# facebookresearch/spdl

Hardware: AMD Instinct MI355X
Metric: images/sec device-resident JPEG→RGB224, 1/2/4/8×MI355X; % HBM roofline (higher is better)
Workload: dtype u8; 1 GPU; configs[1]: synthetic 480x640 q90 4:2:0 baseline JPEG resident in HBM -> RGB 224x224 u8 (scale bicubic decrease + centred pad, rgb24); global_batch=256, per_gpu_batch=256, distinct_images=32, lanes=4, hw_queues=4, entropy_threads=256, entropy_piece_bytes=131072

## Files before the change

### spdl_amd/csrc/hj_host.cpp

```cpp
#include <hip/hip_runtime.h>

#include <algorithm>
#include <cmath>
#include <cstdarg>
#include <cstdio>
#include <cstring>
#include <map>
#include <memory>
#include <string>
#include <vector>

#include "../../include/spdl_hipjpeg.h"
#include "hj_common.h"
#include "hj_launch.h"
#include "hj_layout.h"
#include "hj_pack.h"
#include "hj_probe.h"
#include "hj_sws.h"
#include "hj_tar.h"
#include "hj_views.h"

using namespace hj;

namespace {

constexpr int kStages = 8;
const char* kStageNames[kStages] = {"h2d",  "parse",  "destuff", "entropy",
                                    "idct", "tables", "output",  "d2h_status"};

void set_err(char* err, size_t errlen, const char* fmt, ...) {
  if (!err || !errlen) return;
  va_list ap;
  va_start(ap, fmt);
  vsnprintf(err, errlen, fmt, ap);
  va_end(ap);
}

int plan_batch(const LayoutRequest& rq, Layout& L, int32_t* status, char* err, size_t errlen) {
  const LayoutResult r = build_layout(rq, L);
  if (r.rc) {
    if (status && r.image >= 0) status[r.image] = r.rc;
    set_err(err, errlen, "%s", r.err);
  }
  return r.rc;
}

struct DevBuf {
  void* p = nullptr;
  size_t cap = 0;
  hipError_t ensure(size_t n, hipStream_t st = nullptr, bool async = false) {
    if (n <= cap) return hipSuccess;
// ... 62 lines not shown
  bool profiled = false;
  uint32_t profiled_stages = 0;
  hipEvent_t submitted = nullptr;
  int n = 0;
  hipEvent_t ev[kStages + 1] = {};
  struct Retry {
    int64_t ticket = 0;
    const uint8_t* bytes = nullptr;
    size_t len = 0;
    spdl_hj_output out{};
    uint8_t* out_dev = nullptr;
    struct Item {
      int idx;
      size_t out_off, out_bytes;
      int64_t off, size;
      spdl_hj_image_info info;
      spdl_hj_rect rect;
      uint8_t flip;
      uint8_t lowres;
    };
    std::vector<Item> items;
    bool has_rects = false, has_flips = false;
    bool oriented = false;
  } retry;
};

constexpr int kMaxLanes = 8;

struct Workspace {
  DevBuf clean, segs, desc, info, luts, ents, bdesc, planes, wts, recs, dschunks;
  DevBuf chain;
  DevBuf maps;
  DevBuf hbuf;
  hipEvent_t done = nullptr;
  hipStream_t stream = nullptr;
  hipStream_t side = nullptr;
  hipEvent_t ev_parsed = nullptr, ev_ms = nullptr;
  hipStream_t last_st = nullptr;
  bool used = false;
};

struct spdl_hj_ctx {
  int device = 0;
  Workspace ws[kMaxLanes];
  int lanes = 1;
  Slot slots[kSlots + 1];
  int64_t next_ticket = 1;
  int64_t last_ticket = 0;
  int lanes_ready = 0;
  hipStream_t copy = nullptr;
  CopyPool* pool = nullptr;
  int hw_queues = 4;
  int lane_priority = 1;
  int output_path = 0;
  bool profiling = false;
  uint32_t profile_stages = (1u << kStages) - 1u;
  float timings[kStages] = {};
  int ntimings = 0;
  int sub_bits = 384;
  int debug_mask = 0;
  int host_staging = 1;
  int entropy_threads = 0;
  int warm_slots = -1;
  int64_t piece_bytes = 128 * 1024;
  int min_run_slots = 0;
  int chain_after = -1;
// ... 127 lines not shown
  int first_bad = -1;
  for (int i = 0; i < n; i++) {
    if (status) status[i] = stv[i];
    if (stv[i] != SPDL_HJ_OK && first_bad < 0) first_bad = i;
  }
  if (first_bad >= 0) {
    set_err(err, errlen, "Failed to decode an image. (image %d: %s)", first_bad,
            status_str(stv[first_bad]));
    return stv[first_bad];
  }
  return SPDL_HJ_OK;
}

EntropyParams entropy_schedule(const spdl_hj_ctx* c, int* threads) {
  const int t = *threads = c->entropy_threads ? c->entropy_threads : (c->lanes > 1 ? 256 : 512);
  EntropyParams ep{};
  ep.sub_bits = c->sub_bits;
  ep.warm_slots = c->warm_slots >= 0 ? c->warm_slots : (t <= 256 ? 6 : 12);
  ep.min_run_slots = c->min_run_slots;
  ep.chain_after = c->chain_after >= 0 ? c->chain_after : (t >= 512 ? 1 : 2);
  ep.prio = c->entropy_prio;
  ep.ablate = c->debug_mask & kAblEntropy;
  ep.handoff_ticks = c->handoff_wait_us * 100;
  return ep;
}

template <class T>
hipError_t grow(DevBuf& d, size_t bytes, hipStream_t st, T** p) {
  const hipError_t e = d.ensure(bytes, st, true);
  *p = static_cast<T*>(d.p);
  return e;
}
int workspace_buffers(Workspace& W, const Layout& L, int n, const uint8_t* d_bytes,
                      int64_t max_end, hipStream_t st, BatchBuffers* b, char* err, size_t errlen) {
  b->bytes = d_bytes;
  b->n = n;
  b->ndesc = (int)L.desc.size();
  b->nwork = (int)L.work.size();
  HJ_HIP(grow(W.clean, (size_t)max_end + 512, st, &b->clean));
  HJ_HIP(grow(W.segs, (size_t)L.total_segs * 4 + 64, st, &b->segs));
  HJ_HIP(grow(W.dschunks, (size_t)L.total_ds * sizeof(DsChunk) + 64, st, &b->dschunks));
  HJ_HIP(grow(W.desc,
              sizeof(ImageDesc) * b->ndesc + sizeof(uint32_t) * b->nwork + L.flips.size() +
                  L.lowres.size(),
              st, &b->desc));
  b->work = reinterpret_cast<uint32_t*>(b->desc + b->ndesc);
  b->flips = L.flips.empty() ? nullptr : reinterpret_cast<const uint8_t*>(b->work + b->nwork);
  b->transposed = L.transposed;
  b->lowres = L.lowres.empty()
                  ? nullptr
                  : reinterpret_cast<const uint8_t*>(b->work + b->nwork) + L.flips.size();
  HJ_HIP(grow(W.chain, (size_t)(kChainHead + L.chain_granules) * 8 + 64, st, &b->chain));
  HJ_HIP(grow(W.maps, (size_t)(L.ds_wgs + L.idct_wgs + L.hs_wgs + L.sws_wgs) * 4 + 64, st,
              &b->ds_map));
  b->idct_map = b->ds_map + L.ds_wgs;
  b->hs_map = b->idct_map + L.idct_wgs;
  b->sws_map = b->hs_map + L.hs_wgs;
  HJ_HIP(grow(W.hbuf, (size_t)L.total_hbuf * 2 + 64, st, &b->hbuf));
  HJ_HIP(grow(W.info, sizeof(ImageInfo) * n, st, &b->infos));
  HJ_HIP(grow(W.luts, sizeof(HuffTable) * 8 * n, st, &b->luts));
  HJ_HIP(grow(W.ents, (size_t)L.total_blocks * 256 + 256, st, &b->ents));
  HJ_HIP(grow(W.bdesc, (size_t)L.total_blocks * 8 + 64, st, &b->bdesc));
  HJ_HIP(grow(W.planes, (size_t)L.total_planes + 256, st, &b->planes));
  HJ_HIP(grow(W.recs, (size_t)L.total_recs * 4 + 256, st, &b->recs));
  HJ_HIP(grow(W.wts, L.tables.size() * 4 + 256, st, &b->wts));
  return SPDL_HJ_OK;
}

struct Submission {
  const uint8_t* d_bytes;
  size_t bytes_len;
  int n;
  const spdl_hj_output* out;
  void* out_dev;
  size_t out_bytes;
  hipStream_t st;
  int sync;
  int32_t* status;
  bool planes_only = false;
  const spdl_hj_rect* crops = nullptr;
  const uint8_t* flips = nullptr;
  bool oriented = false;
  const int64_t* ragged = nullptr;
};

void set_chain(BatchParams& p, const spdl_hj_output& o, int w, int h) {
  p.pix_fmt = o.pix_fmt;
  p.dtype = o.dtype;
  p.resize = o.resize;
  p.filter = o.filter;
  p.out_w = w;
// ... 3 lines not shown
}

int run_pipeline(spdl_hj_ctx* ctx, Slot& slot, const Layout& L, const Submission& sub, char* err,
                 size_t errlen) {
  const int n = sub.n;
  const spdl_hj_output* const out = sub.out;
  const hipStream_t st = sub.st;
  const size_t esz = out->dtype == SPDL_HJ_DTYPE_U8 ? 1 : 2;
  const bool by_views = !L.groups.empty();
  if (!sub.planes_only && !by_views && !L.ragged &&
      (size_t)L.out_elems_per_image * n * esz > sub.out_bytes) {
    set_err(err, errlen, "output buffer too small: need %lld bytes, have %zu",
            (long long)(L.out_elems_per_image * n * esz), sub.out_bytes);
    return SPDL_HJ_ERR_INVALID_ARG;
  }
  int64_t max_end = 0;
  for (int i = 0; i < n; i++) {
    if (L.desc[i].in_off % 256) {
      set_err(err, errlen, "image %d offset %lld is not 256-byte aligned", i,
              (long long)L.desc[i].in_off);
      return SPDL_HJ_ERR_INVALID_ARG;
    }
    int64_t e = L.desc[i].in_off + L.desc[i].in_size;
    if (L.desc[i].in_off < 0 || L.desc[i].in_size < 0 || (size_t)e > sub.bytes_len) {
      set_err(err, errlen, "image %d extends past the input buffer", i);
      return SPDL_HJ_ERR_INVALID_ARG;
    }
    if (e > max_end) max_end = e;
  }
  Workspace& W = ctx->ws[slot.ticket % ctx->lanes];
  if (!(ctx->lean_waits && W.used && W.last_st == st)) HJ_HIP(hipStreamWaitEvent(st, W.done, 0));
  W.last_st = st;
  W.used = true;
  BatchBuffers B;
  if (int rc = workspace_buffers(W, L, n, sub.d_bytes, max_end, st, &B, err, errlen)) return rc;
  auto use_flat = [&](int64_t flat_wgs, int64_t max_tiles) {
    return (double)max_tiles * n > 1.25 * (double)flat_wgs;
  };
  const bool ds_flat = use_flat(L.ds_wgs, L.max_chunks);
  const bool idct_flat = B.lowres != nullptr ||
                         use_flat(L.idct_wgs, (L.max_blocks + kIdctThreads - 1) / kIdctThreads);
  const bool sws_flat = use_flat(L.sws_wgs, (int64_t)L.sws_bands * L.sws_chunks);
  const size_t work_end = sizeof(ImageDesc) * B.ndesc + sizeof(uint32_t) * B.nwork;
  const size_t desc_bytes = work_end + L.flips.size() + L.lowres.size();
  HJ_HIP(slot.pin_desc.ensure(desc_bytes));
  HJ_HIP(slot.pin_status.ensure(sizeof(int32_t) * n));
  slot.n = n;
  memcpy(slot.pin_desc.p, L.desc.data(), sizeof(ImageDesc) * B.ndesc);
  memcpy(static_cast<ImageDesc*>(slot.pin_desc.p) + B.ndesc, L.work.data(),
         sizeof(uint32_t) * B.nwork);
  if (B.flips)
    memcpy(static_cast<uint8_t*>(slot.pin_desc.p) + work_end, L.flips.data(), L.flips.size());
  if (B.lowres)
    memcpy(static_cast<uint8_t*>(slot.pin_desc.p) + work_end + L.flips.size(), L.lowres.data(),
           L.lowres.size());
  const bool swscale = !sub.planes_only && out->csc == SPDL_HJ_CSC_SWSCALE;
  const size_t tb = swscale ? L.tables.size() * 4 : 0;
  HJ_HIP(slot.pin_tables.ensure(tb + 16));
  if (tb) memcpy(slot.pin_tables.p, L.tables.data(), tb);
  const bool hs = ctx->host_staging != 0;
  if (!hs) {
    HJ_HIP(hipMemcpyAsync(B.desc, slot.pin_desc.p, desc_bytes, hipMemcpyHostToDevice, st));
    if (tb) HJ_HIP(hipMemcpyAsync(B.wts, slot.pin_tables.p, tb, hipMemcpyHostToDevice, st));
  } else if (B.flips || B.lowres) {
    HJ_HIP(hipMemcpyAsync(reinterpret_cast<uint8_t*>(B.work + B.nwork),
                          static_cast<const uint8_t*>(slot.pin_desc.p) + work_end,
                          desc_bytes - work_end, hipMemcpyHostToDevice, st));
  }
// ... 540 lines not shown
    return nullptr;
  }
  DeviceGuard g(device);
  auto* c = new spdl_hj_ctx();
  c->device = device;
  if (const char* q = getenv("GPU_MAX_HW_QUEUES")) c->hw_queues = atoi(q) > 0 ? atoi(q) : 4;
  bool ok = ensure_lanes(c, 1);
  for (int i = 0; ok && i <= kSlots; i++)
    ok = hipEventCreateWithFlags(&c->slots[i].h2d_done, hipEventDisableTiming) == hipSuccess &&
         hipEventCreateWithFlags(&c->slots[i].done, hipEventDisableTiming) == hipSuccess &&
         hipEventCreateWithFlags(&c->slots[i].submitted, hipEventDisableTiming) == hipSuccess;
  for (int i = 0; ok && i <= kSlots; i++)
    for (int k = 0; ok && k <= kStages; k++) ok = hipEventCreate(&c->slots[i].ev[k]) == hipSuccess;
  if (!ok) {
    set_err(err, errlen, "hipEventCreate / hipStreamCreate failed");
    spdl_hj_destroy(c);
    return nullptr;
  }
  return c;
}

void spdl_hj_destroy(spdl_hj_ctx* c) {
  if (!c) return;
  DeviceGuard g(c->device);
  for (Slot& s : c->slots)
    if (s.ticket && s.done) (void)hipEventSynchronize(s.done);
  for (Workspace& w : c->ws) {
    if (w.done) (void)hipEventSynchronize(w.done);
    if (w.stream) (void)hipStreamSynchronize(w.stream);
  }
  if (c->copy) (void)hipStreamSynchronize(c->copy);
  for (Workspace& w : c->ws) {
    DevBuf* bufs[] = {&w.clean, &w.segs, &w.desc, &w.info, &w.luts, &w.ents, &w.bdesc,
                      &w.planes, &w.wts, &w.recs, &w.dschunks};
    for (DevBuf* b : bufs) b->release();
    if (w.done) (void)hipEventDestroy(w.done);
    if (w.stream) (void)hipStreamDestroy(w.stream);
    if (w.ev_parsed) (void)hipEventDestroy(w.ev_parsed);
    if (w.ev_ms) (void)hipEventDestroy(w.ev_ms);
    if (w.side) (void)hipStreamDestroy(w.side);
  }
  for (Slot& s : c->slots) {
    s.bytes.release();
    s.pin_in.release();
    s.pin_desc.release();
    s.pin_status.release();
    s.pin_tables.release();
    if (s.h2d_done) (void)hipEventDestroy(s.h2d_done);
    if (s.done) (void)hipEventDestroy(s.done);
    if (s.submitted) (void)hipEventDestroy(s.submitted);
    for (int k = 0; k <= kStages; k++)
      if (s.ev[k]) (void)hipEventDestroy(s.ev[k]);
  }
  if (c->copy) (void)hipStreamDestroy(c->copy);
  delete c->pool;
  delete c;
}

int spdl_hj_decode_batch(spdl_hj_ctx* ctx, const uint8_t* const* data, const size_t* sizes,
                         int32_t n, const spdl_hj_output* out, void* out_dev, size_t out_bytes,
                         void* stream, int32_t sync, int32_t* status, char* err, size_t errlen) {
  const Held held(ctx, n, out, out_dev, out_bytes, err, errlen);
  if (int rc = held.check(ctx && data && sizes, n, out, out_dev, err, errlen)) return rc;
  std::vector<int64_t> offs(n), szs(n);
  std::vector<CopyItem> items(n);
  int64_t total = 0;
  for (int i = 0; i < n; i++) {
// ... 543 lines not shown
```

### spdl_amd/csrc/hj_kernels.hip

```cpp
#include <hip/hip_fp16.h>
#include <hip/hip_runtime.h>

#include "hj_common.h"
#include "hj_destuff.h"
#include "hj_idct.h"
#include "hj_launch.h"
#include "hj_sws_tile.h"
#include "hj_upsample.h"

namespace hj {

__device__ __forceinline__ uint32_t rfl(uint32_t v) { return __builtin_amdgcn_readfirstlane(v); }


struct ParseScratch {
  ImageInfo info;
  uint16_t qt[4][64];
  uint8_t bits[8][17];
  uint8_t vals[8][256];
  int32_t have[8];
  int32_t qhave[4];
  int32_t maxcode[8][18];
  int32_t valoff[8][17];
  int32_t dqt_off[4], dqt_pq[4];
// ... 374 lines not shown
    tab_nsub[t] = nsub;
  }
  __syncthreads();
  if (tid == 0) {
    int ns = 0, seen = 0, subs = 0, slow = 0;
    for (int c = 0; c < s.info.ncomp; c++)
      for (int k = 0; k < 2; k++) {
        const int slot = k == 0 ? s.info.dc_tab[c] : 4 + s.info.ac_tab[c];
        if (!(seen & (1 << slot))) {
          ns++;
          subs += tab_nsub[slot];
          slow |= (tab_slow >> slot) & 1;
          slow |= tab_nsub[slot] > (kSubShare >> kSubBits);
        }
        seen |= 1 << slot;
      }
    s.info.ent_wide = !(ns <= 4 && (subs << kSubBits) <= kSubPool && !slow);
  }
  __syncthreads();
  HJ_PT();
#if HJ_PARSE_PROF
  if (tid == 0)
    for (int i = 1; i < npt && i < 8; i++) s.info.sdiag[39 + i] = (int32_t)(pt[i] - pt[0]);
#endif
  static_assert(sizeof(ImageInfo) % 4 == 0, "ImageInfo copied in words");
  {
    const uint32_t* src = reinterpret_cast<const uint32_t*>(&s.info);
    uint32_t* dst = reinterpret_cast<uint32_t*>(infos + img);
    for (int i = tid; i < (int)(sizeof(ImageInfo) / 4); i += blockDim.x) dst[i] = src[i];
  }
}


__global__ void __launch_bounds__(256) lut_kernel(const uint8_t* __restrict__ bytes,
                                                  const ImageDesc* __restrict__ desc,
                                                  ImageInfo* __restrict__ infos,
                                                  HuffTable* __restrict__ luts) {
  __shared__ int first, same, maxcode[18], valoff[17];
  __shared__ uint8_t bits[17], vals[256];
  const int t = blockIdx.x, img = blockIdx.y, tid = threadIdx.x;
  const ImageInfo& in = infos[img];
  if (in.status != kOk || in.multiscan || in.tab_n[t] == 0) return;
  const uint32_t h = in.tab_hash[t];
  const int n = in.tab_n[t];
  const uint8_t* d = bytes + desc[img].in_off + in.tab_off[t];
  if (tid == 0) first = img;
  __syncthreads();
  for (int j = tid; j < img; j += blockDim.x) {
    const ImageInfo& o = infos[j];
    if (o.status == kOk && !o.multiscan && o.tab_n[t] == n && o.tab_hash[t] == h)
      atomicMin(&first, j);
  }
  __syncthreads();
  const int j = first;
  if (j < img) {
    if (tid == 0) same = 1;
    __syncthreads();
    const uint8_t* e = bytes + desc[j].in_off + infos[j].tab_off[t];
    for (int k = tid; k < 16 + n; k += blockDim.x)
      if (d[k] != e[k]) same = 0;
    __syncthreads();
    if (same) {
      if (tid == 0) infos[img].lut_ref[t] = j * 8 + t;
      return;
    }
  }
  if (tid < 16) bits[tid + 1] = d[tid];
  for (int k = tid; k < 256; k += blockDim.x) vals[k] = k < n ? d[16 + k] : 0;
  __syncthreads();
  if (tid == 0) {
    int code = 0, k = 0;
    for (int l = 1; l <= 16; l++) {
// ... 4105 lines not shown
__device__ __forceinline__ void hbuf_stage(const int16_t* __restrict__ src, int w, int rows, int c0,
                                           int ncols, int r0, int r1, int16_t* dst, int cst,
                                           int tid, int nt) {
  const int nr = r1 - r0, ne = ncols * nr;
  for (int i0 = tid; i0 < ne; i0 += 4 * nt) {
    int16_t v[4];
#pragma unroll
    for (int u = 0; u < 4; u++) {
      const int i = min(i0 + u * nt, ne - 1);
      const int r = i / ncols, c = i - r * ncols;
      v[u] = src[(int64_t)min(r0 + r, rows - 1) * w + c0 + c];
    }
#pragma unroll
    for (int u = 0; u < 4; u++) {
      const int i = i0 + u * nt;
      if (i < ne) {
        const int r = i / ncols, c = i - r * ncols;
        dst[c * cst + r] = v[u];
      }
    }
  }
}

template <bool kOrient>
__global__ void __launch_bounds__(256) sws_kernel(const uint8_t* __restrict__ planes,
                                                  const ImageDesc* __restrict__ desc,
                                                  const ImageInfo* __restrict__ infos,
                                                  const int32_t* __restrict__ pool,
                                                  void* __restrict__ out, const BatchParams p,
                                                  int32_t* __restrict__ host_status,
                                                  const int16_t* __restrict__ hbuf,
                                                  const uint32_t* __restrict__ sws_map,
                                                  const int wg0,
                                                  const uint8_t* __restrict__ flips) {
  extern __shared__ __attribute__((aligned(16))) int16_t sws_lds[];
  const bool flat = sws_map != nullptr;
  uint32_t bx = blockIdx.x, by = blockIdx.y, bz = blockIdx.z;
  if (p.xcd_order & 1) xcd_order(bx, by, bz);
  if (flat) bx += (uint32_t)wg0;
  const int img = flat ? (int)sws_map[bx] : (int)bz, tid = threadIdx.x, nt = blockDim.x;
  const ImageDesc& dd = desc[img];
  const int t = flat ? (int)bx - dd.sws_wg0 : (int)(bx * dd.sws_chunks + by);
  const int band = flat ? t / dd.sws_chunks : (int)bx;
  const int chunk = flat ? t - band * dd.sws_chunks : (int)by;
  const ImageInfo& in = infos[dd.src];
  if (host_status && t == 0 && tid == 0) host_status[img] = in.status;
  if (in.status != kOk || dd.refuse) return;
  const SwsDesc& s = dd.sws;
  const int yo0 = band * s.rb, xo0 = chunk * s.col_chunk;
  if (yo0 >= dd.oh || xo0 >= dd.ow) return;
  const SwsWindow win =
      sws_window(yo0, xo0, s.rb, s.col_chunk, dd.dx, dd.dy, dd.ow, dd.oh, s.sw, s.sh);
  const int yo1 = win.yo1, xo1 = win.xo1, th = yo1 - yo0, tw = xo1 - xo0;
  const int ys0 = win.ys0, ys1 = win.ys1, xs0 = win.xs0, xs1 = win.xs1;
  const bool content = win.content;
  const int flip = flips ? __builtin_amdgcn_readfirstlane((int)flips[img]) : 0;
  const TileFlip tf = tile_flip(xo0, xo1, yo0, yo1, dd.ow, dd.oh, flip);
  TileOrient to{};
  int lw = 0, lh = 0, fw = 0, mx0 = 0, my0 = 0;
  if constexpr (kOrient) {
    to = tile_orient(xo0, xo1, yo0, yo1, dd.ow, dd.oh, flip);
    lw = to.lw;
    lh = to.lh;
    fw = to.fw;
    mx0 = to.mx0();
    my0 = to.my0();
  }
  const bool planar = p.pix_fmt == 0 || p.pix_fmt == 1;
  const bool swap = p.pix_fmt == 1 || p.pix_fmt == 3;
  const bool u8 = p.dtype == 0;
  const int64_t pl = (int64_t)dd.ow * dd.oh;
  const int32_t* T = pool + dd.wt_off;
  const int32_t* vl_pos = T + s.off[kVlPos];
  const int32_t* vc_pos = T + s.off[kVcPos];
  int lr0 = 0, lr1 = 0, cr0 = 0, cr1 = 0;
  SwsChromaCols ccols = {0, 0};
  const int ncl = content ? xs1 - xs0 : 0;
  if (content) {
    lr0 = vl_pos[ys0];
    lr1 = vl_pos[ys1 - 1] + s.vl_taps;
    if (!s.gray) {
      cr0 = vc_pos[ys0];
      cr1 = vc_pos[ys1 - 1] + s.vc_taps;
      ccols = sws_chroma_cols(xs0, xs1, s.full);
    }
  }
  const int cx0 = ccols.cx0, ncc = ccols.ncc;
  const SwsLds lay = sws_lds_layout(ncl, ncc, lr1 - lr0, cr1 - cr0, s.gbr, s.gray, s.rb,
                                    s.col_chunk, s.vl_size, s.vc_size);
  const int lst = lay.lst, cst = lay.cst, vrw = lay.vrw;
  int16_t *hl = sws_lds, *hu = hl + lay.hu, *hv = hl + lay.hv;
  uint8_t* tile = reinterpret_cast<uint8_t*>(sws_lds) + lay.tile;
  uint32_t* vt = reinterpret_cast<uint32_t*>(reinterpret_cast<uint8_t*>(sws_lds) + lay.vt);
  if (content) {
    const int32_t* vmode = T + s.off[kVmode];
    const uint32_t* vlw = reinterpret_cast<const uint32_t*>(T + s.off[kVlCoef]);
    const uint32_t* vcw = reinterpret_cast<const uint32_t*>(T + s.off[kVcCoef]);
    const int nl = s.vl_size / 2, nc = s.vc_size / 2;
    for (int i = tid; i < (ys1 - ys0) * vrw; i += nt) {
      const int r = i / vrw, w = i - r * vrw, ys = ys0 + r;
      uint32_t v = 0;
      if (w == 0) v = (uint32_t)vmode[ys];
      else if (w == 1) v = (uint32_t)(vl_pos[ys] - lr0);
      else if (w == 2) v = s.gray ? 0u : (uint32_t)(vc_pos[ys] - cr0);
      else if (w >= 4 && w < 4 + nl) v = vlw[(int64_t)ys * nl + (w - 4)];
      else if (w >= 4 + nl) v = vcw[(int64_t)ys * nc + (w - 4 - nl)];
      vt[i] = v;
    }
  }
  auto putc = [&](int xo, int yo, int c0v, int c1v, int c2v) {
    const int cv[3] = {c0v, c1v, c2v};
    int tx, ty;
    if constexpr (kOrient) {
      tx = to.lx(xo, yo);
      ty = to.ly(xo, yo);
    } else {
      tx = tf.tx(xo);
      ty = tf.ty(yo);
    }
    if (u8) {
#pragma unroll
      for (int ch = 0; ch < 3; ch++) {
        const int v = cv[ch];
        int ti;
        if constexpr (kOrient) ti = planar ? (ch * lh + ty) * lw + tx : (ty * lw + tx) * 3 + ch;
        else ti = planar ? (ch * th + ty) * tw + tx : (ty * tw + tx) * 3 + ch;
        tile[ti] = (uint8_t)v;
      }
      return;
    }
    const int mx = (kOrient ? mx0 : tf.mx0) + tx, my = (kOrient ? my0 : tf.my0) + ty;
#pragma unroll
    for (int ch = 0; ch < 3; ch++) {
      const int v = cv[ch];
      int64_t oi;
      if constexpr (kOrient)
        oi = dd.out_off + (planar ? ch * pl + (int64_t)my * fw + mx : ((int64_t)my * fw + mx) * 3 + ch);
      else
        oi = dd.out_off + (planar ? ch * pl + (int64_t)my * dd.ow + mx : ((int64_t)my * dd.ow + mx) * 3 + ch);
      float f = __fdiv_rn((float)v, 255.0f);
      f = __fsub_rn(f, p.mean[ch]);
      f = __fdiv_rn(f, p.std[ch]);
      static_cast<uint16_t*>(out)[oi] = to_f16_bits(f, p.dtype);
    }
  };
  auto put = [&](int xo, int yo, const int* rgb) {
    putc(xo, yo, swap ? rgb[2] : rgb[0], rgb[1], swap ? rgb[0] : rgb[2]);
  };
  {
    const int cy0 = content ? ys0 + dd.dy : yo1, cy1 = content ? ys1 + dd.dy : yo1;
    const int cxa = xs0 + dd.dx, cxb = xs1 + dd.dx;
    if (cy0 > yo0 || cy1 < yo1 || cxa > xo0 || cxb < xo1) {
      const int lane = tid & 63, nw = nt >> 6;
      const int wave = __builtin_amdgcn_readfirstlane(tid >> 6);
      auto zrun = [&](int off, int n, int t, int nth) {
        const int head = min(n, -off & 3), words = (n - head) >> 2;
        const int tail = n - head - 4 * words;
        uint8_t* q = tile + off + head;
        if (t < head) tile[off + t] = 0;
        for (int i = t; i < words; i += nth) reinterpret_cast<uint32_t*>(q)[i] = 0u;
        if (t < tail) q[4 * words + t] = 0;
      };
      auto fill = [&](int ya, int yb, int xa, int xb) {
        if (ya >= yb || xa >= xb) return;
        if (!u8) {
          for (int yo = ya + wave; yo < yb; yo += nw)
            for (int xo = xa + lane; xo < xb; xo += 64) putc(xo, yo, 0, 0, 0);
          return;
        }
        const int bpp = planar ? 1 : 3, np_ = planar ? 3 : 1;
        const int ps = th * tw;
        if constexpr (kOrient) {
          const int k0 = min(to.lx(xa, ya), to.lx(xb - 1, yb - 1));
          const int r0 = min(to.ly(xa, ya), to.ly(xb - 1, yb - 1));
          const int kw = to.t ? yb - ya : xb - xa, rh = to.t ? xb - xa : yb - ya;
          if (kw == lw) {
            for (int pc = 0; pc < np_; pc++) zrun((pc * ps + r0 * lw) * bpp, rh * lw * bpp, tid, nt);
            return;
          }
          for (int r = r0 + wave; r < r0 + rh; r += nw)
            for (int pc = 0; pc < np_; pc++) zrun((pc * ps + r * lw + k0) * bpp, kw * bpp, lane, 64);
          return;
        }
        const int r0 = min(tf.ty(ya), tf.ty(yb - 1)), k0 = min(tf.tx(xa), tf.tx(xb - 1));
        if (xb - xa == tw) {
          for (int pc = 0; pc < np_; pc++)
            zrun((pc * ps + r0 * tw) * bpp, (yb - ya) * tw * bpp, tid, nt);
          return;
        }
        for (int yo = ya + wave; yo < yb; yo += nw)
          for (int pc = 0; pc < np_; pc++)
            zrun((pc * ps + tf.ty(yo) * tw + k0) * bpp, (xb - xa) * bpp, lane, 64);
      };
      fill(yo0, cy0, xo0, xo1);
      fill(cy1, yo1, xo0, xo1);
      fill(cy0, cy1, xo0, cxa);
      fill(cy0, cy1, cxb, xo1);
    }
  }
  if (content && s.pre) {
    const int16_t* hb = hbuf + dd.hbuf_off;
    hbuf_stage(hb, s.sw, s.pre_rl, xs0, ncl, lr0, lr1, hl, lst, tid, nt);
    if (s.gbr || !s.gray) {
      const HsPlane p1 = hs_plane(s, 1), p2 = hs_plane(s, 2);
      const int c0 = s.gbr ? xs0 : cx0, nc = s.gbr ? ncl : ncc;
      const int q0 = s.gbr ? lr0 : cr0, q1 = s.gbr ? lr1 : cr1, st = s.gbr ? lst : cst;
      hbuf_stage(hb + p1.off, p1.w, p1.rows, c0, nc, q0, q1, hu, st, tid, nt);
      hbuf_stage(hb + p2.off, p2.w, p2.rows, c0, nc, q0, q1, hv, st, tid, nt);
    }
  } else if (content && s.gbr) {
    const int third = nt / 3, c = min(tid / third, 2), t3 = tid - c * third;
    if (tid < 3 * third)
      hpass(win_rows(planes, dd, c), dd.plane_stride[c], dd.win_h[c], dd.win_x[c],
            T + s.off[kHlPos],
            reinterpret_cast<const int16_t*>(T + s.off[kHlCoef]), s.hl_size, s.hl_taps, xs0, ncl,
            lr0, lr1, c == 0 ? hl : c == 1 ? hu : hv, lst, t3, third);
  } else if (content && !(p.debug_mask & kAblSwsHpass)) {
    hpass(win_rows(planes, dd, 0), dd.plane_stride[0], dd.win_h[0], dd.win_x[0],
          T + s.off[kHlPos],
          reinterpret_cast<const int16_t*>(T + s.off[kHlCoef]), s.hl_size, s.hl_taps, xs0, ncl,
          lr0, lr1, hl, lst, tid, nt);
    if (!s.gray) {
      const int half = nt >> 1, t2 = tid < half ? tid : tid - half;
      const int c = tid < half ? 1 : 2;
      hpass(win_rows(planes, dd, c), dd.plane_stride[c], dd.win_h[c], dd.win_x[c],
            T + s.off[kHcPos],
            reinterpret_cast<const int16_t*>(T + s.off[kHcCoef]), s.hc_size, s.hc_taps, cx0, ncc,
            cr0, cr1, c == 1 ? hu : hv, cst, t2, half);
    }
  }
// ... 809 lines not shown
      vmax = max(vmax, dd.v_samp[c]);
    }
  }
  int v[3][2][8];
#pragma unroll
  for (int c = 0; c < 3; c++) {
    if (c < dd.ncomp) {
      const int hr = dd.ncomp > 1 ? hmax / dd.h_samp[c] : 1;
      const int vr = dd.ncomp > 1 ? vmax / dd.v_samp[c] : 1;
      const int cw = dd.win_w[c], ch = dd.win_h[c];
      up::run8x2(planes + dd.plane_off[c], dd.plane_stride[c], cw, ch, up::mode_of(hr, vr, cw), hr,
                 vr, x0, y0, v[c][0], v[c][1]);
    } else {
#pragma unroll
      for (int k = 0; k < 8; k++) {
        v[c][0][k] = v[0][0][k];
        v[c][1][k] = v[0][1][k];
      }
    }
  }
  turbo_row(out, dd, p, x0, y0, v[0][0], v[1][0], v[2][0]);
  if (y0 + 1 < H) turbo_row(out, dd, p, x0, y0 + 1, v[0][1], v[1][1], v[2][1]);
}


hipError_t launch_parse(const BatchBuffers& b, const ImageDesc* host_desc, const void* host_tables,
                        int64_t table_bytes, int threads, hipStream_t st) {
  const auto* host_work =
      host_desc ? reinterpret_cast<const uint32_t*>(host_desc + b.ndesc) : nullptr;
  hipLaunchKernelGGL(parse_kernel, dim3(b.n), dim3(threads), 0, st, b.bytes, host_desc, b.desc,
                     b.infos, b.luts, static_cast<const uint4*>(host_tables),
                     reinterpret_cast<uint4*>(b.wts), (table_bytes + 15) / 16, host_work, b.work,
                     b.nwork, b.chain, b.ds_map, b.idct_map, b.hs_map, b.sws_map, b.ndesc);
  hipLaunchKernelGGL(lut_kernel, dim3(8, b.n), dim3(256), 0, st, b.bytes, b.desc, b.infos, b.luts);
  return hipGetLastError();
}
hipError_t launch_destuff(const BatchBuffers& b, bool flat, int ds_wgs, int max_chunks,
                          hipStream_t st) {
  const dim3 grid = flat ? dim3(ds_wgs) : dim3(max_chunks, b.n);
  const uint32_t* map = flat ? b.ds_map : nullptr;
  hipLaunchKernelGGL(destuff_count_kernel, grid, dim3(kDsThreads), 0, st, b.bytes, b.desc, b.infos,
                     b.dschunks, map);
  hipLaunchKernelGGL(destuff_prefix_kernel, dim3(b.n), dim3(kDsThreads), 0, st, b.desc, b.infos,
                     b.dschunks);
  hipLaunchKernelGGL(destuff_write_kernel, grid, dim3(kDsThreads), 0, st, b.bytes, b.desc, b.infos,
                     b.dschunks, b.clean, b.segs, map);
  return hipGetLastError();
}
hipError_t launch_entropy(const BatchBuffers& b, const EntropyParams& ep, int threads, int lds_pad,
                          hipStream_t st) {
#define HJ_ENT(T, NTAB)                                                                        \
  hipLaunchKernelGGL((entropy_kernel<T, NTAB>), dim3(b.nwork), dim3(T), lds_pad, st, b.clean,  \
                     b.segs, b.desc, b.infos, b.luts, b.ents, b.bdesc, b.recs, b.work, b.chain, \
                     ep, b.nwork)
  switch (threads) {
    case 1024: HJ_ENT(1024, 4); break;
    case 512: HJ_ENT(512, 4); break;
    case 128: HJ_ENT(128, 4); break;
    default: HJ_ENT(256, 4);
  }
#undef HJ_ENT
  return hipGetLastError();
}
hipError_t launch_multiscan(const BatchBuffers& b, hipStream_t st) {
  hipLaunchKernelGGL(multiscan_kernel, dim3(b.n), dim3(256), 0, st, b.bytes, b.clean, b.desc,
                     b.infos, b.ents, b.bdesc);
  return hipGetLastError();
// ... 44 lines not shown
  const int gx = (int)std::min<int64_t>((max_px / 4 + 255) / 256 + 1, 1024);
  hipLaunchKernelGGL(cmyk_kernel, dim3(gx, b.n), dim3(256), 0, st, b.desc, b.infos, b.planes);
  return hipGetLastError();
}
hipError_t launch_csc(const BatchBuffers& b, void* out, const BatchParams& p, int64_t max_px,
                      int32_t* host_status, hipStream_t st) {
  const int gx = (int)std::min<int64_t>((max_px + 255) / 256, 4096);
  hipLaunchKernelGGL(csc_kernel, dim3(gx, b.n), dim3(256), 0, st, b.planes, b.desc, b.infos, out, p,
                     host_status);
  return hipGetLastError();
}
hipError_t launch_turbo_rgb(const BatchBuffers& b, void* out, const BatchParams& p, int turbo_wgs,
                            int32_t* host_status, hipStream_t st) {
  hipLaunchKernelGGL(turbo_rgb_kernel, dim3(turbo_wgs), dim3(256), 0, st, b.planes, b.desc, b.infos,
                     out, p, host_status, b.sws_map);
  return hipGetLastError();
}
hipError_t launch_rgb_unscaled(const BatchBuffers& b, void* out, const BatchParams& p,
                               int64_t max_px, int32_t* host_status, hipStream_t st) {
  const int64_t groups = (max_px + kRgbPx - 1) / kRgbPx + 64;
  const int gx = (int)std::min<int64_t>((groups + 255) / 256, 1024);
  hipLaunchKernelGGL(rgb_unscaled_kernel, dim3(gx, b.n), dim3(256), 0, st, b.planes, b.desc,
                     b.infos, static_cast<uint8_t*>(out), p, host_status);
  return hipGetLastError();
}
static void launch_hscale(const BatchBuffers& b, int hs_wgs, hipStream_t st) {
  if (hs_wgs > 0)
    hipLaunchKernelGGL(hscale_kernel, dim3(hs_wgs), dim3(256), 0, st, b.planes, b.desc, b.infos,
                       b.wts, b.hs_map, b.hbuf);
}
hipError_t launch_sws(const BatchBuffers& b, void* out, const BatchParams& p, bool flat,
                      int sws_wgs, int bands, int chunks, int lds_bytes, int hs_wgs,
                      int32_t* host_status, hipStream_t st, int wg0) {
  launch_hscale(b, hs_wgs, st);
  const dim3 grid = flat ? dim3(sws_wgs) : dim3(bands, chunks, b.n);
  hipLaunchKernelGGL(b.transposed ? sws_kernel<true> : sws_kernel<false>, grid, dim3(256), lds_bytes,
                     st, b.planes, b.desc, b.infos, b.wts, out, p, host_status, b.hbuf,
                     flat ? b.sws_map : nullptr, wg0, b.flips);
  return hipGetLastError();
}
hipError_t launch_yuv_planes(const BatchBuffers& b, void* out, int sws_wgs, int lds_bytes,
                             int hs_wgs, int32_t* host_status, hipStream_t st) {
  launch_hscale(b, hs_wgs, st);
  hipLaunchKernelGGL(yuv_planes_kernel, dim3(sws_wgs), dim3(256), lds_bytes, st, b.planes, b.desc,
                     b.infos, b.wts, static_cast<uint8_t*>(out), host_status, b.hbuf, b.sws_map,
                     b.flips);
  return hipGetLastError();
}

}
```

### spdl_amd/csrc/hj_launch.h

```cpp
#pragma once
#include <hip/hip_runtime.h>

#include "hj_common.h"

namespace hj {

struct BatchBuffers {
  const uint8_t* bytes;
  uint8_t *clean, *planes;
  uint32_t *segs, *ents, *recs;
  uint32_t* work;
  DsChunk* dschunks;
  ImageDesc* desc;
  ImageInfo* infos;
  HuffTable* luts;
  uint2* bdesc;
  uint64_t* chain;
  int32_t* wts;
  int16_t* hbuf;
  uint32_t *ds_map, *idct_map, *hs_map, *sws_map;
  int n, nwork;
  int ndesc;
  const uint8_t* flips;
  bool transposed;
  const uint8_t* lowres;
};

hipError_t launch_parse(const BatchBuffers& b, const ImageDesc* host_desc, const void* host_tables,
                        int64_t table_bytes, int threads, hipStream_t st);
hipError_t launch_destuff(const BatchBuffers& b, bool flat, int ds_wgs, int max_chunks,
                          hipStream_t st);
hipError_t launch_entropy(const BatchBuffers& b, const EntropyParams& ep, int threads, int lds_pad,
                          hipStream_t st);
hipError_t launch_multiscan(const BatchBuffers& b, hipStream_t st);
hipError_t launch_idct(const BatchBuffers& b, int idct, bool flat, int idct_wgs, int max_blocks,
                       int xcd, hipStream_t st);
hipError_t launch_idct_lowres(const BatchBuffers& b, int idct, int idct_wgs, hipStream_t st);
hipError_t launch_cmyk(const BatchBuffers& b, int64_t max_px, hipStream_t st);
hipError_t launch_csc(const BatchBuffers& b, void* out, const BatchParams& p, int64_t max_px,
                      int32_t* host_status, hipStream_t st);
hipError_t launch_turbo_rgb(const BatchBuffers& b, void* out, const BatchParams& p, int turbo_wgs,
                            int32_t* host_status, hipStream_t st);
hipError_t launch_rgb_unscaled(const BatchBuffers& b, void* out, const BatchParams& p,
                               int64_t max_px, int32_t* host_status, hipStream_t st);
hipError_t launch_idct_rgb(const BatchBuffers& b, void* out, const BatchParams& p, int idct,
                           int tiles, int32_t* host_status, hipStream_t st);
hipError_t launch_idct_rgb_flat(const BatchBuffers& b, void* out, const BatchParams& p, int idct,
                                int fused_wgs, int32_t* host_status, hipStream_t st);
hipError_t launch_sws(const BatchBuffers& b, void* out, const BatchParams& p, bool flat,
                      int sws_wgs, int bands, int chunks, int lds_bytes, int hs_wgs,
                      int32_t* host_status, hipStream_t st, int wg0 = 0);
hipError_t launch_yuv_planes(const BatchBuffers& b, void* out, int sws_wgs, int lds_bytes,
                             int hs_wgs, int32_t* host_status, hipStream_t st);
// ... 5 lines not shown
```

### spdl_amd/csrc/hj_sws_tile.h

```cpp
#pragma once
#include "hj_common.h"

namespace hj {

inline HJ_HD int tile_min(int a, int b) { return a < b ? a : b; }
inline HJ_HD int tile_max(int a, int b) { return a > b ? a : b; }
inline HJ_HD int tile_div_up(int a, int b) { return (a + b - 1) / b; }
inline HJ_HD int tile_align16(int v) { return (v + 15) & ~15; }

struct SwsWindow {
  int yo1, xo1, ys0, ys1, xs0, xs1;
  bool content;
};
inline HJ_HD SwsWindow sws_window(int yo0, int xo0, int rb, int col_chunk, int dx, int dy, int ow,
                                  int oh, int sw, int sh) {
  const int yo1 = tile_min(yo0 + rb, oh), xo1 = tile_min(xo0 + col_chunk, ow);
  const int ys0 = tile_max(yo0 - dy, 0), ys1 = tile_min(yo1 - dy, sh);
  const int xs0 = tile_max(xo0 - dx, 0), xs1 = tile_min(xo1 - dx, sw);
  return {yo1, xo1, ys0, ys1, xs0, xs1, ys0 < ys1 && xs0 < xs1};
}

struct TileFlip {
  int mx0, my0;
  int xm, xb, ym, yb;
// ... 18 lines not shown
  HJ_HD int lx(int xo, int yo) const { return f.tx(t ? yo : xo); }
  HJ_HD int ly(int xo, int yo) const { return f.ty(t ? xo : yo); }
  HJ_HD int cx(int kx, int ky) const { return t ? f.sy(ky) : f.sx(kx); }
  HJ_HD int cy(int kx, int ky) const { return t ? f.sx(kx) : f.sy(ky); }
};
inline HJ_HD TileOrient tile_orient(int xo0, int xo1, int yo0, int yo1, int ow, int oh, int code) {
  const bool t = code & 4;
  const int fw = t ? oh : ow, fh = t ? ow : oh;
  const TileFlip f = t ? tile_flip(yo0, yo1, xo0, xo1, fw, fh, code & 3)
                       : tile_flip(xo0, xo1, yo0, yo1, fw, fh, code & 3);
  return {f, t, fw, fh, t ? yo1 - yo0 : xo1 - xo0, t ? xo1 - xo0 : yo1 - yo0};
}

struct SwsChromaCols {
  int cx0, ncc;
};
inline HJ_HD SwsChromaCols sws_chroma_cols(int xs0, int xs1, bool full) {
  const int cx0 = full ? xs0 : xs0 >> 1;
  return {cx0, (full ? xs1 - 1 : (xs1 - 1) >> 1) + 1 - cx0};
}

struct SwsLds {
  int lst, cst, hu, hv, tile, vt, vrw, end;
};
inline HJ_HD SwsLds sws_lds_layout(int ncl, int ncc, int lrows, int crows, bool gbr, bool gray,
                                   int rb, int col_chunk, int vl_size, int vc_size) {
  const int lst = sws_col_stride(lrows), cst = sws_col_stride(crows);
  const int side = gbr ? ncl * lst : gray ? 0 : ncc * cst;
  const int hu = ncl * lst, hv = hu + side, tile = tile_align16(2 * (hv + side));
  const int vt = tile + tile_align16(rb * col_chunk * 3), vrw = 4 + (vl_size + vc_size) / 2;
  return {lst, cst, hu, hv, tile, vt, vrw, vt + rb * vrw * 4};
}

struct PlanarLds {
  int cst, tile, pitch, bound;
};
inline HJ_HD PlanarLds planar_lds_layout(int ncols, int rows, int rb, int chunk) {
  const int cst = sws_col_stride(rows), tile = tile_align16(2 * ncols * cst);
  const int pitch = (chunk + 30) & ~15;
  return {cst, tile, pitch, tile + rb * pitch + 16};
}

struct HsTiles {
  int tl, tc, wgs;
};
inline HJ_HD HsTiles hs_tiles(const SwsDesc& s) {
  const int tl = tile_div_up(s.pre_rl, kHsRows);
  const int tc = s.gbr ? tl : s.gray ? 0 : tile_div_up(s.pre_rc, kHsRows);
  return {tl, tc, tl + 2 * tc};
}
struct HsPlane {
  int64_t off;
  int rows, w;
};
inline HJ_HD HsPlane hs_plane(const SwsDesc& s, int c) {
  const bool lumaf = c == 0 || s.gbr;
  const int64_t side = s.gbr ? (int64_t)s.pre_rl * s.sw : (int64_t)s.pre_rc * s.chr_w;
  return {c == 0 ? 0 : (int64_t)s.pre_rl * s.sw + (c - 1) * side, lumaf ? s.pre_rl : s.pre_rc,
          lumaf ? s.sw : s.chr_w};
}
inline HJ_HD int64_t hs_hbuf_size(const SwsDesc& s) {
  const HsPlane last = hs_plane(s, hs_tiles(s).tc ? 2 : 0);
  return last.off + (int64_t)last.rows * last.w;
}

struct PlanarTiles {
// ... 12 lines not shown
```

Before: 612,600 images/sec.

## Precompute per-tile swscale records and vertical tables in the LUT kernel

```diff
diff --git a/spdl_amd/csrc/hj_host.cpp b/spdl_amd/csrc/hj_host.cpp
--- a/spdl_amd/csrc/hj_host.cpp
+++ b/spdl_amd/csrc/hj_host.cpp
@@ -17,6 +17,7 @@
 #include "hj_pack.h"
 #include "hj_probe.h"
 #include "hj_sws.h"
+#include "hj_sws_tile.h"
 #include "hj_tar.h"
 #include "hj_views.h"
 
@@ -145,6 +146,7 @@
   DevBuf chain;
   DevBuf maps;
   DevBuf hbuf;
+  DevBuf tiles;
   hipEvent_t done = nullptr;
   hipStream_t stream = nullptr;
   hipStream_t side = nullptr;
@@ -338,7 +340,8 @@
   return e;
 }
 int workspace_buffers(Workspace& W, const Layout& L, int n, const uint8_t* d_bytes,
-                      int64_t max_end, hipStream_t st, BatchBuffers* b, char* err, size_t errlen) {
+                      int64_t max_end, int tile_wg0, hipStream_t st, BatchBuffers* b, char* err,
+                      size_t errlen) {
   b->bytes = d_bytes;
   b->n = n;
   b->ndesc = (int)L.desc.size();
@@ -363,6 +366,18 @@
   b->hs_map = b->idct_map + L.idct_wgs;
   b->sws_map = b->hs_map + L.hs_wgs;
   HJ_HIP(grow(W.hbuf, (size_t)L.total_hbuf * 2 + 64, st, &b->hbuf));
+  b->tiles = nullptr;
+  b->tile_slot16 = 0;
+  b->tile_wg0 = std::max(tile_wg0, 0);
+  b->sws_wgs = (int)L.sws_wgs;
+  if (tile_wg0 >= 0 && L.sws_wgs > tile_wg0) {
+    int vt_words = 0;
+    for (const ImageDesc& d : L.desc)
+      if (sws_tiled(d))
+        vt_words = std::max(vt_words, d.sws.rb * (4 + (d.sws.vl_size + d.sws.vc_size) / 2));
+    b->tile_slot16 = sws_tile_slot16(vt_words);
+    HJ_HIP(grow(W.tiles, (size_t)L.sws_wgs * b->tile_slot16 * 16 + 64, st, &b->tiles));
+  }
   HJ_HIP(grow(W.info, sizeof(ImageInfo) * n, st, &b->infos));
   HJ_HIP(grow(W.luts, sizeof(HuffTable) * 8 * n, st, &b->luts));
   HJ_HIP(grow(W.ents, (size_t)L.total_blocks * 256 + 256, st, &b->ents));
@@ -432,8 +447,16 @@
   if (!(ctx->lean_waits && W.used && W.last_st == st)) HJ_HIP(hipStreamWaitEvent(st, W.done, 0));
   W.last_st = st;
   W.used = true;
+  const bool sws_generic =
+      !sub.planes_only && !(ctx->debug_mask & kAblNoOutput) && out->csc != SPDL_HJ_CSC_TURBO &&
+      (by_views || L.ragged ||
+       (out->csc == SPDL_HJ_CSC_SWSCALE && out->pix_fmt != SPDL_HJ_FMT_YUV &&
+        !(L.all_special && out->dtype == SPDL_HJ_DTYPE_U8 && ctx->output_path != 1)));
   BatchBuffers B;
-  if (int rc = workspace_buffers(W, L, n, sub.d_bytes, max_end, st, &B, err, errlen)) return rc;
+  if (int rc = workspace_buffers(W, L, n, sub.d_bytes, max_end,
+                                 sws_generic ? (L.ragged ? (int)L.fused_wgs : 0) : -1, st, &B, err,
+                                 errlen))
+    return rc;
   auto use_flat = [&](int64_t flat_wgs, int64_t max_tiles) {
     return (double)max_tiles * n > 1.25 * (double)flat_wgs;
   };
@@ -1040,7 +1063,7 @@
   if (c->copy) (void)hipStreamSynchronize(c->copy);
   for (Workspace& w : c->ws) {
     DevBuf* bufs[] = {&w.clean, &w.segs, &w.desc, &w.info, &w.luts, &w.ents, &w.bdesc,
-                      &w.planes, &w.wts, &w.recs, &w.dschunks};
+                      &w.planes, &w.wts, &w.recs, &w.dschunks, &w.tiles};
     for (DevBuf* b : bufs) b->release();
     if (w.done) (void)hipEventDestroy(w.done);
     if (w.stream) (void)hipStreamDestroy(w.stream);
diff --git a/spdl_amd/csrc/hj_kernels.hip b/spdl_amd/csrc/hj_kernels.hip
--- a/spdl_amd/csrc/hj_kernels.hip
+++ b/spdl_amd/csrc/hj_kernels.hip
@@ -430,12 +430,60 @@
 }
 
 
+struct SwsTileRec16 {
+  uint4 q[kSwsTileRecWords / 4];
+};
+__device__ __forceinline__ void write_tiles(const ImageDesc* __restrict__ desc,
+                                            const int32_t* __restrict__ pool,
+                                            const uint32_t* __restrict__ sws_map,
+                                            uint4* __restrict__ tiles, int slot16, int wg0,
+                                            int sws_wgs, int ndesc, int wg, int nwg, int tid,
+                                            int nt) {
+  for (int64_t g = (int64_t)wg0 + wg; g < sws_wgs; g += nwg) {
+    uint4* slot = tiles + g * slot16;
+    const uint32_t img = sws_map[g];
+    const ImageDesc& dd = desc[img < (uint32_t)ndesc ? img : 0u];
+    const int64_t t = g - dd.sws_wg0;
+    if (img >= (uint32_t)ndesc || !sws_tiled(dd) || t < 0 ||
+        t >= (int64_t)dd.sws_bands * dd.sws_chunks) {
+      if (tid == 0) slot[0] = make_uint4(0u, 0u, 0u, 0u);
+      continue;
+    }
+    const SwsDesc& s = dd.sws;
+    const int32_t* T = pool + dd.wt_off;
+    const int band = (int)t / dd.sws_chunks, chunk = (int)t - band * dd.sws_chunks;
+    const SwsTileRec r = sws_tile_rec(dd, T, band, chunk);
+    if (tid == 0) {
+      const SwsTileRec16 r16 = __builtin_bit_cast(SwsTileRec16, r);
+#pragma unroll
+      for (int q = 0; q < kSwsTileRecWords / 4; q++) slot[q] = r16.q[q];
+    }
+    uint32_t* vt = reinterpret_cast<uint32_t*>(slot) + kSwsTileRecWords;
+    const int nvt = min(r.nvt, 4 * slot16 - kSwsTileRecWords);
+    for (int v = tid; v < nvt; v += nt) {
+      const int row = v / r.vrw, w = v - row * r.vrw;
+      vt[v] = sws_vt_word(s, T, r.ys0 + row, w, r.lr0, r.cr0);
+    }
+  }
+}
+
 __global__ void __launch_bounds__(256) lut_kernel(const uint8_t* __restrict__ bytes,
                                                   const ImageDesc* __restrict__ desc,
                                                   ImageInfo* __restrict__ infos,
-                                                  HuffTable* __restrict__ luts) {
+                                                  HuffTable* __restrict__ luts,
+                                                  const int32_t* __restrict__ pool,
+                                                  const uint32_t* __restrict__ sws_map,
+                                                  uint4* __restrict__ tiles, const int slot16,
+                                                  const int tile_wg0, const int sws_wgs,
+                                                  const int ndesc) {
   __shared__ int first, same, maxcode[18], valoff[17];
   __shared__ uint8_t bits[17], vals[256];
+  if (blockIdx.x >= 8) {
+    write_tiles(desc, pool, sws_map, tiles, slot16, tile_wg0, sws_wgs, ndesc,
+                (int)((blockIdx.x - 8) * gridDim.y + blockIdx.y), (int)((gridDim.x - 8) * gridDim.y),
+                (int)threadIdx.x, (int)blockDim.x);
+    return;
+  }
   const int t = blockIdx.x, img = blockIdx.y, tid = threadIdx.x;
   const ImageInfo& in = infos[img];
   if (in.status != kOk || in.multiscan || in.tab_n[t] == 0) return;
@@ -4607,7 +4655,9 @@
                                                   const int16_t* __restrict__ hbuf,
                                                   const uint32_t* __restrict__ sws_map,
                                                   const int wg0,
-                                                  const uint8_t* __restrict__ flips) {
+                                                  const uint8_t* __restrict__ flips,
+                                                  const uint4* __restrict__ tiles,
+                                                  const int slot16) {
   extern __shared__ __attribute__((aligned(16))) int16_t sws_lds[];
   const bool flat = sws_map != nullptr;
   uint32_t bx = blockIdx.x, by = blockIdx.y, bz = blockIdx.z;
@@ -4616,19 +4666,18 @@
   const int img = flat ? (int)sws_map[bx] : (int)bz, tid = threadIdx.x, nt = blockDim.x;
   const ImageDesc& dd = desc[img];
   const int t = flat ? (int)bx - dd.sws_wg0 : (int)(bx * dd.sws_chunks + by);
-  const int band = flat ? t / dd.sws_chunks : (int)bx;
-  const int chunk = flat ? t - band * dd.sws_chunks : (int)by;
   const ImageInfo& in = infos[dd.src];
   if (host_status && t == 0 && tid == 0) host_status[img] = in.status;
   if (in.status != kOk || dd.refuse) return;
   const SwsDesc& s = dd.sws;
-  const int yo0 = band * s.rb, xo0 = chunk * s.col_chunk;
-  if (yo0 >= dd.oh || xo0 >= dd.ow) return;
-  const SwsWindow win =
-      sws_window(yo0, xo0, s.rb, s.col_chunk, dd.dx, dd.dy, dd.ow, dd.oh, s.sw, s.sh);
-  const int yo1 = win.yo1, xo1 = win.xo1, th = yo1 - yo0, tw = xo1 - xo0;
-  const int ys0 = win.ys0, ys1 = win.ys1, xs0 = win.xs0, xs1 = win.xs1;
-  const bool content = win.content;
+  if (!flat && ((int)bx >= dd.sws_bands || (int)by >= dd.sws_chunks)) return;
+  const uint4* slot = tiles + (int64_t)(flat ? (int)bx : dd.sws_wg0 + t) * slot16;
+  const SwsTileRec& R = *reinterpret_cast<const SwsTileRec*>(slot);
+  if (!R.valid) return;
+  const int yo0 = R.yo0, xo0 = R.xo0;
+  const int yo1 = R.yo1, xo1 = R.xo1, th = yo1 - yo0, tw = xo1 - xo0;
+  const int ys0 = R.ys0, ys1 = R.ys1, xs0 = R.xs0;
+  const bool content = R.content != 0;
   const int flip = flips ? __builtin_amdgcn_readfirstlane((int)flips[img]) : 0;
   const TileFlip tf = tile_flip(xo0, xo1, yo0, yo1, dd.ow, dd.oh, flip);
   TileOrient to{};
@@ -4646,42 +4695,17 @@
   const bool u8 = p.dtype == 0;
   const int64_t pl = (int64_t)dd.ow * dd.oh;
   const int32_t* T = pool + dd.wt_off;
-  const int32_t* vl_pos = T + s.off[kVlPos];
-  const int32_t* vc_pos = T + s.off[kVcPos];
-  int lr0 = 0, lr1 = 0, cr0 = 0, cr1 = 0;
-  SwsChromaCols ccols = {0, 0};
-  const int ncl = content ? xs1 - xs0 : 0;
+  const int lr0 = R.lr0, lr1 = R.lr1, cr0 = R.cr0, cr1 = R.cr1;
+  const int ncl = R.ncl, cx0 = R.cx0, ncc = R.ncc;
+  const int lst = R.lst, cst = R.cst, vrw = R.vrw;
+  int16_t *hl = sws_lds, *hu = hl + R.hu, *hv = hl + R.hv;
+  uint8_t* tile = reinterpret_cast<uint8_t*>(sws_lds) + R.tile;
+  uint32_t* vt = reinterpret_cast<uint32_t*>(reinterpret_cast<uint8_t*>(sws_lds) + R.vt);
   if (content) {
-    lr0 = vl_pos[ys0];
-    lr1 = vl_pos[ys1 - 1] + s.vl_taps;
-    if (!s.gray) {
-      cr0 = vc_pos[ys0];
-      cr1 = vc_pos[ys1 - 1] + s.vc_taps;
-      ccols = sws_chroma_cols(xs0, xs1, s.full);
-    }
-  }
-  const int cx0 = ccols.cx0, ncc = ccols.ncc;
-  const SwsLds lay = sws_lds_layout(ncl, ncc, lr1 - lr0, cr1 - cr0, s.gbr, s.gray, s.rb,
-                                    s.col_chunk, s.vl_size, s.vc_size);
-  const int lst = lay.lst, cst = lay.cst, vrw = lay.vrw;
-  int16_t *hl = sws_lds, *hu = hl + lay.hu, *hv = hl + lay.hv;
-  uint8_t* tile = reinterpret_cast<uint8_t*>(sws_lds) + lay.tile;
-  uint32_t* vt = reinterpret_cast<uint32_t*>(reinterpret_cast<uint8_t*>(sws_lds) + lay.vt);
-  if (content) {
-    const int32_t* vmode = T + s.off[kVmode];
-    const uint32_t* vlw = reinterpret_cast<const uint32_t*>(T + s.off[kVlCoef]);
-    const uint32_t* vcw = reinterpret_cast<const uint32_t*>(T + s.off[kVcCoef]);
-    const int nl = s.vl_size / 2, nc = s.vc_size / 2;
-    for (int i = tid; i < (ys1 - ys0) * vrw; i += nt) {
-      const int r = i / vrw, w = i - r * vrw, ys = ys0 + r;
-      uint32_t v = 0;
-      if (w == 0) v = (uint32_t)vmode[ys];
-      else if (w == 1) v = (uint32_t)(vl_pos[ys] - lr0);
-      else if (w == 2) v = s.gray ? 0u : (uint32_t)(vc_pos[ys] - cr0);
-      else if (w >= 4 && w < 4 + nl) v = vlw[(int64_t)ys * nl + (w - 4)];
-      else if (w >= 4 + nl) v = vcw[(int64_t)ys * nc + (w - 4 - nl)];
-      vt[i] = v;
-    }
+    const uint4* src = slot + kSwsTileRecWords / 4;
+    const int n4 = R.nvt >> 2, rest = R.nvt & 3;
+    for (int i = tid; i < n4; i += nt) reinterpret_cast<uint4*>(vt)[i] = src[i];
+    if (tid < rest) vt[4 * n4 + tid] = reinterpret_cast<const uint32_t*>(src)[4 * n4 + tid];
   }
   auto putc = [&](int xo, int yo, int c0v, int c1v, int c2v) {
     const int cv[3] = {c0v, c1v, c2v};
@@ -4723,9 +4747,7 @@
     putc(xo, yo, swap ? rgb[2] : rgb[0], rgb[1], swap ? rgb[0] : rgb[2]);
   };
   {
-    const int cy0 = content ? ys0 + dd.dy : yo1, cy1 = content ? ys1 + dd.dy : yo1;
-    const int cxa = xs0 + dd.dx, cxb = xs1 + dd.dx;
-    if (cy0 > yo0 || cy1 < yo1 || cxa > xo0 || cxb < xo1) {
+    if (R.npad) {
       const int lane = tid & 63, nw = nt >> 6;
       const int wave = __builtin_amdgcn_readfirstlane(tid >> 6);
       auto zrun = [&](int off, int n, int t, int nth) {
@@ -4767,10 +4789,8 @@
           for (int pc = 0; pc < np_; pc++)
             zrun((pc * ps + tf.ty(yo) * tw + k0) * bpp, (xb - xa) * bpp, lane, 64);
       };
-      fill(yo0, cy0, xo0, xo1);
-      fill(cy1, yo1, xo0, xo1);
-      fill(cy0, cy1, xo0, cxa);
-      fill(cy0, cy1, cxb, xo1);
+#pragma unroll
+      for (int k = 0; k < 4; k++) fill(R.pad[k].ya, R.pad[k].yb, R.pad[k].xa, R.pad[k].xb);
     }
   }
   if (content && s.pre) {
@@ -5646,7 +5666,14 @@
                      b.infos, b.luts, static_cast<const uint4*>(host_tables),
                      reinterpret_cast<uint4*>(b.wts), (table_bytes + 15) / 16, host_work, b.work,
                      b.nwork, b.chain, b.ds_map, b.idct_map, b.hs_map, b.sws_map, b.ndesc);
-  hipLaunchKernelGGL(lut_kernel, dim3(8, b.n), dim3(256), 0, st, b.bytes, b.desc, b.infos, b.luts);
+  int tile_cols = 0;
+  if (b.tiles) {
+    const int64_t ntiles = b.sws_wgs - b.tile_wg0;
+    tile_cols = (int)std::clamp<int64_t>((ntiles + 2LL * b.n - 1) / (2LL * b.n), 1, 1024);
+  }
+  hipLaunchKernelGGL(lut_kernel, dim3(8 + tile_cols, b.n), dim3(256), 0, st, b.bytes, b.desc,
+                     b.infos, b.luts, b.wts, b.sws_map, b.tiles, b.tile_slot16, b.tile_wg0,
+                     b.sws_wgs, b.ndesc);
   return hipGetLastError();
 }
 hipError_t launch_destuff(const BatchBuffers& b, bool flat, int ds_wgs, int max_chunks,
@@ -5757,11 +5784,12 @@
 hipError_t launch_sws(const BatchBuffers& b, void* out, const BatchParams& p, bool flat,
                       int sws_wgs, int bands, int chunks, int lds_bytes, int hs_wgs,
                       int32_t* host_status, hipStream_t st, int wg0) {
+  if (!b.tiles) return hipErrorInvalidValue;
   launch_hscale(b, hs_wgs, st);
   const dim3 grid = flat ? dim3(sws_wgs) : dim3(bands, chunks, b.n);
   hipLaunchKernelGGL(b.transposed ? sws_kernel<true> : sws_kernel<false>, grid, dim3(256), lds_bytes,
                      st, b.planes, b.desc, b.infos, b.wts, out, p, host_status, b.hbuf,
-                     flat ? b.sws_map : nullptr, wg0, b.flips);
+                     flat ? b.sws_map : nullptr, wg0, b.flips, b.tiles, b.tile_slot16);
   return hipGetLastError();
 }
 hipError_t launch_yuv_planes(const BatchBuffers& b, void* out, int sws_wgs, int lds_bytes,
diff --git a/spdl_amd/csrc/hj_launch.h b/spdl_amd/csrc/hj_launch.h
--- a/spdl_amd/csrc/hj_launch.h
+++ b/spdl_amd/csrc/hj_launch.h
@@ -19,6 +19,8 @@
   int32_t* wts;
   int16_t* hbuf;
   uint32_t *ds_map, *idct_map, *hs_map, *sws_map;
+  uint4* tiles;
+  int tile_slot16, tile_wg0, sws_wgs;
   int n, nwork;
   int ndesc;
   const uint8_t* flips;
diff --git a/spdl_amd/csrc/hj_sws_tile.h b/spdl_amd/csrc/hj_sws_tile.h
--- a/spdl_amd/csrc/hj_sws_tile.h
+++ b/spdl_amd/csrc/hj_sws_tile.h
@@ -74,6 +74,83 @@
   return {lst, cst, hu, hv, tile, vt, vrw, vt + rb * vrw * 4};
 }
 
+inline HJ_HD bool sws_tiled(const ImageDesc& d) {
+  const SwsDesc& s = d.sws;
+  return !d.refuse && !s.yuv && s.rb > 0 && s.col_chunk > 0 && d.sws_bands > 0 && d.sws_chunks > 0 &&
+         d.sws_bands == tile_div_up(d.oh, s.rb) && d.sws_chunks == tile_div_up(d.ow, s.col_chunk);
+}
+
+struct SwsPadRect {
+  int32_t ya, yb, xa, xb;
+};
+struct SwsTileRec {
+  int32_t valid;
+  int32_t yo0, xo0;
+  int32_t yo1, xo1, ys0, ys1, xs0, xs1, content;
+  int32_t lr0, lr1, cr0, cr1;
+  int32_t cx0, ncc;
+  int32_t lst, cst, hu, hv, tile, vt, vrw, end;
+  int32_t ncl, nvt, npad;
+  SwsPadRect pad[4];
+  int32_t fill_[5];
+};
+constexpr int kSwsTileRecWords = 48;
+static_assert(sizeof(SwsTileRec) == 4 * kSwsTileRecWords, "SwsTileRec: 48 words");
+
+inline HJ_HD SwsTileRec sws_tile_rec(const ImageDesc& d, const int32_t* T, int band, int chunk) {
+  const SwsDesc& s = d.sws;
+  SwsTileRec r{};
+  r.valid = 1;
+  r.yo0 = band * s.rb;
+  r.xo0 = chunk * s.col_chunk;
+  const SwsWindow w = sws_window(r.yo0, r.xo0, s.rb, s.col_chunk, d.dx, d.dy, d.ow, d.oh, s.sw, s.sh);
+  r.yo1 = w.yo1, r.xo1 = w.xo1, r.ys0 = w.ys0, r.ys1 = w.ys1, r.xs0 = w.xs0, r.xs1 = w.xs1;
+  r.content = w.content;
+  SwsChromaCols cc = {0, 0};
+  if (w.content) {
+    const int32_t* vl_pos = T + s.off[kVlPos];
+    r.ncl = w.xs1 - w.xs0;
+    r.lr0 = vl_pos[w.ys0];
+    r.lr1 = vl_pos[w.ys1 - 1] + s.vl_taps;
+    if (!s.gray) {
+      const int32_t* vc_pos = T + s.off[kVcPos];
+      r.cr0 = vc_pos[w.ys0];
+      r.cr1 = vc_pos[w.ys1 - 1] + s.vc_taps;
+      cc = sws_chroma_cols(w.xs0, w.xs1, s.full);
+    }
+  }
+  r.cx0 = cc.cx0, r.ncc = cc.ncc;
+  const SwsLds l = sws_lds_layout(r.ncl, r.ncc, r.lr1 - r.lr0, r.cr1 - r.cr0, s.gbr, s.gray, s.rb,
+                                  s.col_chunk, s.vl_size, s.vc_size);
+  r.lst = l.lst, r.cst = l.cst, r.hu = l.hu, r.hv = l.hv, r.tile = l.tile, r.vt = l.vt;
+  r.vrw = l.vrw, r.end = l.end;
+  r.nvt = w.content ? (w.ys1 - w.ys0) * l.vrw : 0;
+  const int cy0 = w.content ? w.ys0 + d.dy : w.yo1, cy1 = w.content ? w.ys1 + d.dy : w.yo1;
+  const int cxa = w.xs0 + d.dx, cxb = w.xs1 + d.dx;
+  r.pad[0] = {r.yo0, cy0, r.xo0, w.xo1};
+  r.pad[1] = {cy1, w.yo1, r.xo0, w.xo1};
+  r.pad[2] = {cy0, cy1, r.xo0, cxa};
+  r.pad[3] = {cy0, cy1, cxb, w.xo1};
+  r.npad = (r.pad[0].ya < r.pad[0].yb && r.pad[0].xa < r.pad[0].xb) +
+           (r.pad[1].ya < r.pad[1].yb && r.pad[1].xa < r.pad[1].xb) +
+           (r.pad[2].ya < r.pad[2].yb && r.pad[2].xa < r.pad[2].xb) +
+           (r.pad[3].ya < r.pad[3].yb && r.pad[3].xa < r.pad[3].xb);
+  return r;
+}
+
+inline HJ_HD uint32_t sws_vt_word(const SwsDesc& s, const int32_t* T, int ys, int w, int lr0,
+                                  int cr0) {
+  const int nl = s.vl_size / 2, nc = s.vc_size / 2;
+  if (w == 0) return (uint32_t)T[s.off[kVmode] + ys];
+  if (w == 1) return (uint32_t)(T[s.off[kVlPos] + ys] - lr0);
+  if (w == 2) return s.gray ? 0u : (uint32_t)(T[s.off[kVcPos] + ys] - cr0);
+  if (w < 4) return 0u;
+  if (w < 4 + nl) return (uint32_t)T[s.off[kVlCoef] + (int64_t)ys * nl + (w - 4)];
+  return (uint32_t)T[s.off[kVcCoef] + (int64_t)ys * nc + (w - 4 - nl)];
+}
+
+inline HJ_HD int sws_tile_slot16(int vt_words) { return (kSwsTileRecWords + vt_words + 3) / 4; }
+
 struct PlanarLds {
   int cst, tile, pitch, bound;
 };
```

Result: slower. 603,400 images/sec (-1.5%).
